# bistromath/gr-ais

Hardware: AMD Instinct MI355X
Metric: complex MS/s through corr_est->msk_timing chain; corr_est %HBM roofline (higher is better)
Workload: dtype f32

## Files before the change

__graft_entry__.py:

```python
import os
import subprocess
import sys

ROOT = os.path.dirname(os.path.abspath(__file__))
for _p in (ROOT, os.path.join(ROOT, "gr-ais_amd"), os.path.join(ROOT, "tests")):
    if _p not in sys.path:
        sys.path.insert(0, _p)


def build():
    env = dict(os.environ)
    subprocess.check_call(["make", "-C", os.path.join(ROOT, "gr-ais_amd")], env=env)
    subprocess.check_call(["make", "-C", os.path.join(ROOT, "oracle")], env=env)
    subprocess.check_call(["make", "-C", os.path.join(ROOT, "tests", "emul")], env=env)
    subprocess.check_call(["make", "-C", os.path.join(ROOT, "tests", "emul_hdlc")], env=env)
    subprocess.check_call(["make", "-C", os.path.join(ROOT, "tests", "emul_nmea")], env=env)
    subprocess.check_call(["make", "-C", os.path.join(ROOT, "tests", "emul_msg")], env=env)
    subprocess.check_call(["make", "-C", os.path.join(ROOT, "tests", "emul_xlate")], env=env)
    subprocess.check_call(["make", "-C", os.path.join(ROOT, "tests", "emul_xlate_fmt")], env=env)
    ub = os.path.join(ROOT, "tools", "ubench")
    src, exe = os.path.join(ub, "hbm_ceiling.hip"), os.path.join(ub, "hbm_ceiling")
    if not os.path.exists(exe) or os.path.getmtime(exe) < os.path.getmtime(src):
        subprocess.check_call([os.environ.get("HIPCC", "/opt/rocm/bin/hipcc"), "--offload-arch=gfx950", "-O3", "-o", exe, src], env=env)
    import ais_amd
    from ais_amd import _lib

    assert _lib.lib().aisx_version() >= 300


def smoke():
    import numpy as np
    import torch

    assert torch.cuda.is_available(), "smoke() needs cuda:0"
    import ais_amd
    import oracle_py as orc
    import synth
    from parity import assert_tags_match

    sps, nchan, T = 4, 8, 8192
    tmpl = ais_amd.modulate_vector_bc(ais_amd.gmsk_mod(sps, 0.4), [1, 1, 0, 0] * 7, [1])
    xs = np.stack([synth.make_channel(31 + c, T, "S", sps, amp=1.0, cfo_max=10.0)[0] for c in range(nchan)])
    opts = dict(samples_per_symbol=sps, bits_per_sec=9600.0, clockrec_gain=0.04, omega_relative_limit=0.01,
                fftlen=1024)
    dem = ais_amd.ais_demod(opts, nchan=nchan, max_items=T, stages="core", preamble_symbols=tmpl)
    r = dem.work(torch.as_tensor(xs).cuda())
    prod = r["produced"].cpu().numpy()
    bits = r["bits"].cpu().numpy()
    tags = dem.preamble_detect.tags()
    ndet = 0
    for c in range(nchan):
        ob, _, ot = orc.Demod(sps, tmpl, stages=0).step(xs[c])
        ndet += assert_tags_match(tags[tags["chan"] == c], ot)
        assert prod[c] == len(ob) and np.array_equal(bits[c, : prod[c]], ob)
    fs = ais_amd.square_and_fft_sync_cc(38400.0, 9600.0, 1024, nchan=nchan, max_items=T)
    agc = ais_amd.feedforward_agc_cc(512, 2.0, nchan=nchan, max_items=T + 1024)
    y = ais_amd.freq_sync_agc(fs, agc, torch.as_tensor(xs).cuda())[0].cpu().numpy()
    for c in range(nchan):
        yo, _ = orc.FreqSync(38400.0, 9600.0, 1024).process(xs[c])
        assert np.array_equal(y[c].view(np.uint32), orc.Agc(512, 2.0).work(yo).view(np.uint32))
    print("smoke ok: %d channels, %d detections, %d bits and %d front-end samples identical to the oracle"
          % (nchan, ndet, int(prod.sum()), y.size))


if __name__ == "__main__":
    build()
    if len(sys.argv) > 1 and sys.argv[1] == "smoke":
        smoke()
```

gr-ais_amd/csrc/k_msk.h:

```cpp
#pragma once
#include "aisx_common.h"

namespace aisx {

enum {
    MSK_ST_INTERP_RANGE = 1,
    MSK_ST_CARRY_OVERFLOW = 2,
    MSK_ST_TAGCARRY_OVERFLOW = 4,
    MSK_ST_OUT_FULL = 8,
    MSK_ST_TAGS_TRUNCATED = 16
};
constexpr int MSK_CTN_TRUNC = 0x40000000;
constexpr int MSK_CTN_WILD = 0x20000000;
constexpr int MSK_TAG_TRIPS = 6;

constexpr int MSK_T = 64;
constexpr int MSK_RING = 256;
constexpr int MSK_SLOTS = MSK_RING + 8;
constexpr int MSK_CHUNK = 64;
constexpr int MSK_OFF = 192;
constexpr int MSK_CARRY_MAX = 128;
constexpr int MSK_PAIRS_MAX = 16;
constexpr int MSK_TAPS_PITCH = 12;
constexpr int msk_lds_ring(int lpw) { return MSK_SLOTS * lpw * 8; }
constexpr int MSK_ZERO_ROW = 129;
constexpr int MSK_LDS_MMSE = ((130 * MSK_TAPS_PITCH * 4 + 511) / 512) * 512;
constexpr int MSK_TAGQ = 36;
#ifndef MSK_WAVES_LPW4
#define MSK_WAVES_LPW4 4
#endif
constexpr int msk_waves(int lpw) { return lpw >= 16 ? 64 / lpw : (lpw == 4 ? MSK_WAVES_LPW4 : 4); }
constexpr int msk_wg_channels(int lpw) { return msk_waves(lpw) * lpw; }
constexpr int MSK_STAGE = 32;
static_assert(MSK_STAGE >= 15 + MSK_PAIRS_MAX + 1, "a lock-step run and a general step between two flushes");
constexpr bool msk_staged(int lpw) { return lpw <= 8; }
constexpr int msk_lds_stage(int lpw) { return msk_staged(lpw) ? MSK_STAGE * lpw * 8 : 0; }
constexpr int msk_lds_ringoff(int lpw) { return msk_waves(lpw) * msk_lds_stage(lpw); }
constexpr int msk_lds_wave(int lpw) { return msk_lds_ring(lpw) + MSK_TAGQ * lpw * 8 + lpw * 8; }
constexpr int msk_lds_taboff(int lpw) { return msk_lds_ringoff(lpw) + msk_waves(lpw) * msk_lds_wave(lpw); }
constexpr int msk_lds_bytes(int lpw) { return msk_lds_taboff(lpw) + MSK_LDS_MMSE; }
static_assert(msk_lds_bytes(4) <= 160 * 1024 && msk_lds_bytes(8) <= 160 * 1024 && msk_lds_bytes(16) <= 160 * 1024 &&
              msk_lds_bytes(32) <= 160 * 1024 && msk_lds_bytes(64) <= 160 * 1024, "a workgroup's LDS");
static_assert(msk_lds_bytes(8) + 71680 <= 160 * 1024, "timing recovery + one correlator workgroup per CU");
constexpr int BT_T = 256;
constexpr int BT_SEG = BT_T * 8;

constexpr int MSKP_SMAX = 64;
enum { MSKP_KIND_NONE = 0, MSKP_KIND_NEXT = 1, MSKP_KIND_HANDOFF = 2 };
struct mskp_rst {
    int jA;
    int relA, relB;
    int q0, cap;
    int pad[3];
};
struct mskp_snap {
    int a;
    float mu, omega;
    int div;
    cf y;
    cf nl;
    int cur;
    int cnt;
};
struct mskp_res {
    mskp_snap end;
    cf ay, anl;
    int kind;
    int status;
};
struct mskp_piece {
    int out0, src0, cnt;
};
AISX_HD bool mskp_same_bits(cf a, cf b)
{
    unsigned ar, ai, br, bi;
    __builtin_memcpy(&ar, &a.re, 4);
    __builtin_memcpy(&ai, &a.im, 4);
    __builtin_memcpy(&br, &b.re, 4);
    __builtin_memcpy(&bi, &b.im, 4);
    return ar == br && ai == bi;
}

struct msk_ctag { int rel; float val; };

struct __attribute__((packed, aligned(8))) cf_pair { cf a, b; };

struct MskParams {
    int nchan;
    float d_sps, gain, gain_omega, limit;
    int osps;
    float* mu; float* omega; int* div;
    cf* dly1; cf* dly2; cf* diff1;
    unsigned long long* nread;
    const cf* in; long in_stride; int n;
    const cf* carry_in; cf* carry_out; const int* carry_len_in; int* carry_len_out; int carry_cap;
    int stream_mode; int gr_ninput; int gr_noutput;
    const msk_ctag* ct; const int* ct_n; int ct_cap;
    tag_rec* ctag_out; int* ctag_n_out; int ctag_cap;
    cf* syms; float* err; float* mu_out; long out_stride; int out_cap;
    int* produced; int* consumed; int* status;
    const float* mmse;
    int lds_tab_off;
    int lds_wave_stride, tq_stride, tq_private;
    int lds_ring_off;
    int sym_al16;
    int lpw;
    int inline_tags;
    int max_noutput;
    int ff;
    const int* nrst; const mskp_rst* rst; const mskp_res* res;
    mskp_piece* pieces; int* npieces;
    const int* ct_nc;
};

struct BitTailParams {
    int nchan;
    const cf* syms; long sym_stride;
    const int* produced;
    unsigned char* bits; long bit_stride;
    const cf* prev_sym_in; const unsigned char* prev_bit_in;
    cf* prev_sym_out; unsigned char* prev_bit_out;
    const float* atan_tab;
};

AISX_HD int msk_forecast(float d_sps, int noutput_items)
{
    return (int)ceil((noutput_items * d_sps * 2) + 3.0 * d_sps + 8u);
}

#ifdef MSK_EMU_STATS
extern long msk_stats[8];
#endif
template <class Ctx, bool AUX, bool OSPS2, int LPW, bool FFT = false>
AISX_DI void msk_body(Ctx& cx, const MskParams& p)
{
    static_assert(!FFT || (!AUX && !OSPS2), "the join build has no err / mu ports and osps == 1");
    constexpr int SLOT_B = LPW * 8;
    constexpr int SLOT_SH = LPW == 64 ? 9 : (LPW == 32 ? 8 : (LPW == 16 ? 7 : (LPW == 8 ? 6 : 5)));
    static_assert(LPW == 4 || LPW == 8 || LPW == 16 || LPW == 32 || LPW == 64, "channels per wave");
    typedef unsigned long long u64;
    static_assert(64 % LPW == 0, "whole waves");
    constexpr int NQ = 64 / LPW;
    constexpr int QS = MSK_CHUNK / NQ;
    const int wv = cx.tid() >> 6;
    const int l = cx.tid() & (LPW - 1);
    const int q = (cx.tid() & 63) / LPW;
    const bool owner = q == 0;
    const int cbase = cx.bx() * msk_wg_channels(LPW) + wv * LPW;
    const int c = cbase + l;
    const bool live = c < p.nchan;
    const int cc = live ? c : (p.nchan - 1);

    char* const lds0 = cx.lds();
    char* const lds = lds0 + p.lds_ring_off + wv * p.lds_wave_stride;
    cf* ring = (cf*)lds;
    float* mm = (float*)(lds0 + p.lds_tab_off);
    cf* myring = ring + l;

    for (int i = cx.tid(); i < 129 * 8; i += cx.nthreads())
        mm[(i >> 3) * MSK_TAPS_PITCH + (i & 7)] = p.mmse[i];
    if (cx.tid() < MSK_TAPS_PITCH)
        mm[MSK_ZERO_ROW * MSK_TAPS_PITCH + cx.tid()] = 0.f;
    if (cbase >= p.nchan) {
        cx.sync();
        return;
    }

    const float d_sps = p.d_sps;
    float d_mu = p.mu[cc], d_omega = p.omega[cc];
    int d_div = p.div[cc];
    cf last_interp = p.dly1[cc];
    cf d_dly_diff_1 = p.diff1[cc];
    cf prev_sq = cmul_exact(p.dly2[cc], p.dly2[cc]);
    const unsigned long long R = p.nread[cc];
    int status = 0;
    const int n = p.n;

    const cf* cin = p.carry_in + (long)cc * p.carry_cap;
    int pending = p.carry_len_in[cc];
    if (pending > MSK_CARRY_MAX)
        pending = MSK_CARRY_MAX;
    const int navail = pending + n;
    for (int q = -1; q < pending; q++) {
        const int slot = (q - pending + MSK_OFF) & (MSK_RING - 1);
        myring[slot * LPW] = cin[q + 1];
        if (slot < 8)
            myring[(MSK_RING + slot) * LPW] = cin[q + 1];
    }

    const msk_ctag* ctl = p.ct + (long)cc * p.ct_cap;
    int ntot = p.ct_n[cc];
    if (ntot & MSK_CTN_TRUNC)
        status |= MSK_ST_TAGS_TRUNCATED;
    const bool tame_tags = p.inline_tags && cx.ballot((ntot & MSK_CTN_WILD) != 0) == 0ull;
    ntot &= MSK_CTN_WILD - 1;
    if (ntot > p.ct_cap)
        ntot = p.ct_cap;
    typedef msk_ctag tq_ent;
    tq_ent* const tq = (tq_ent*)(lds + msk_lds_ring(LPW)) + (p.tq_private ? (cx.tid() & 63) : l);
    const int TQS = p.tq_stride;
    const int TQ_NONE = 0x7fffffff;
    int gq = 0;
    int qhead = 0, qn = 0;
    auto tq_fill = [&]() {
        if (qn > 0) {
            tq[0] = tq[(qn - 1) * TQS];
            qn = 1;
        }
        qhead = qn;
        while (qn < MSK_TAGQ && gq < ntot) {
            tq_ent t[4];
#pragma unroll
            for (int j = 0; j < 4; j++)
                t[j] = ctl[gq + j < ntot ? gq + j : ntot - 1];
#pragma unroll
            for (int j = 0; j < 4; j++) {
                if (qn < MSK_TAGQ && gq < ntot) {
                    gq++;
                    tq[qn * TQS] = t[j];
                    qn++;
                }
            }
        }
    };
    int fr_rel = TQ_NONE;
    float nt_val = 0.f;
    int nt_rel = 0x7fffffff;
    auto tq_front = [&]() {
        if (qhead >= qn && gq < ntot)
            tq_fill();
        if (qhead < qn) {
            const tq_ent e = tq[qhead * TQS];
            fr_rel = e.rel;
            nt_val = e.val;
        } else {
            fr_rel = TQ_NONE;
        }
    };
    auto tq_pop = [&]() {
        qhead++;
        tq_front();
    };
    tq_fill();

    constexpr bool FF = FFT;
    bool fin_saved = false;
    float fin_mu = 0.f, fin_omega = 0.f;
    int fin_div = 0, fin_status = 0;
    cf fin_interp = mk(0.f, 0.f), fin_diff = mk(0.f, 0.f);
    unsigned fin_worst = 0;
    int ffK = 0, ffnck = 0, cand = 0, candj = 0x7fffffff, ffnp = 0;
    int voff = 0;
    const mskp_rst* const ffrs = FF ? p.rst + (long)cc * MSKP_SMAX : nullptr;
    const mskp_res* const ffrr = FF ? p.res + (long)cc * MSKP_SMAX : nullptr;
    if (FF) {
        ffnck = p.ct_nc[cc];
        ffK = ffnck >= 0 ? p.nrst[cc] : 0;
        candj = ffK > 0 ? ffrs[0].jA + 1 + ffnck : 0x7fffffff;
    }

    char* const osym0 = (char*)(p.syms + (long)cbase * p.out_stride);
    char* const oerr0 = AUX && p.err ? (char*)(p.err + (long)cbase * p.out_stride) : nullptr;
    char* const omu0 = AUX && p.mu_out ? (char*)(p.mu_out + (long)cbase * p.out_stride) : nullptr;
    unsigned ob = (unsigned)((long)(cc - cbase) * p.out_stride) * 8u;
    constexpr bool STG = !AUX && !OSPS2 && msk_staged(LPW);
    constexpr unsigned FLQ = NQ < 8 ? NQ : 8;
    constexpr unsigned FL = 2 * FLQ;
    constexpr unsigned STG_MASK = (unsigned)((MSK_STAGE - 1) * SLOT_B);
    const unsigned obrow = ob;
    const unsigned stg_real = (unsigned)(wv * msk_lds_stage(LPW) + l * 8);
    const unsigned stg_spare = (unsigned)(p.lds_ring_off + wv * p.lds_wave_stride + p.lds_wave_stride - SLOT_B + l * 8);
    unsigned so = 0;
    unsigned nf = 0;
    struct alignas(8) cf8s { float re, im; };
    auto stage_put = [&](unsigned mask, unsigned base, cf v) {
        cf8s t;
        t.re = v.re;
        t.im = v.im;
        *(cf8s*)(lds0 + ((so & mask) | base)) = t;
        so += (unsigned)SLOT_B;
    };
    auto stage_get = [&](unsigned k) -> cf {
        const cf8s t = *(const cf8s*)(lds0 + ((((k & (unsigned)(MSK_STAGE - 1)) << SLOT_SH)) | stg_real));
        return mk(t.re, t.im);
    };
    auto flush_syms = [&]() {
        if constexpr (STG) {
            if (cx.ballot((so >> SLOT_SH) - nf >= FL) == 0ull)
                return;
            cx.wave_sync();
            while (cx.ballot((so >> SLOT_SH) - nf >= FL) != 0ull) {
                if ((so >> SLOT_SH) - nf >= FL) {
                    const unsigned k0 = nf + 2u * (unsigned)q;
                    if ((NQ <= 8 || (unsigned)q < FLQ) && !fin_saved) {
                        const cf a = stage_get(k0), b = stage_get(k0 + 1u);
                        cf* dst = (cf*)(osym0 + obrow) + k0;
                        if (p.sym_al16) {
                            st16(dst, a, b);
                        } else {
                            st8(dst, a);
                            st8(dst + 1, b);
                        }
                    }
                    nf += FL;
                }
            }
            cx.wave_sync();
        }
    };

    int base = 0, ototal = 0;
    int iidx = 0, oidx = 0;
    int ninp = 0, noutput = 0;
    bool done = false;
    auto setup_round = [&]() {
        int ninput;
        if (p.stream_mode) {
            ninput = (navail - base) - 1;
            noutput = 0;
            if (ninput > 0) {
                noutput = (int)((ninput - 3.0 * d_sps - 8) / (2.0 * d_sps)) + 2;
                while (noutput > 0 && msk_forecast(d_sps, noutput) > ninput)
                    noutput--;
            }
            if (p.max_noutput > 0 && noutput > p.max_noutput)
                noutput = p.max_noutput;
            if (noutput > p.out_cap - ototal) {
                noutput = p.out_cap - ototal;
                status |= MSK_ST_OUT_FULL;
            }
        } else {
            ninput = p.gr_ninput;
            noutput = p.gr_noutput;
        }
        ninp = (int)(ninput - 3.0 * d_sps);
        iidx = 0;
        oidx = 0;
        if (ninp <= 0 || noutput <= 0) {
            done = true;
            return;
        }
        qhead = 0;
        tq_front();
        while (fr_rel < base)
            tq_pop();
        nt_rel = (fr_rel != TQ_NONE && fr_rel - base < ninp) ? fr_rel - base : 0x7fffffff;
    };
    if (!done)
        setup_round();
    const int jump_margin = (int)ceilf(d_sps) + 1;

    const int nchunks = (n + 8 + MSK_CHUNK - 1) / MSK_CHUNK;
    cf r[QS];
    const cf* myin = p.in + (long)cc * p.in_stride;
    auto issue_chunk = [&](int t) {
        const int s0 = t * MSK_CHUNK + q * QS + voff;
        const bool inside = FF ? cx.ballot(!(s0 >= 0 && t * MSK_CHUNK + MSK_CHUNK + voff <= n)) == 0ull : (t * MSK_CHUNK + MSK_CHUNK <= n);
        if (inside) {
            const cf_pair* src = (const cf_pair*)(myin + s0);
#pragma unroll
            for (int k = 0; k < QS / 2; k++) {
                const cf_pair v = src[k];
                r[2 * k] = v.a;
                r[2 * k + 1] = v.b;
            }
        } else {
#pragma unroll
            for (int k = 0; k < QS; k++) {
                r[k] = mk(0.f, 0.f);
                if (s0 + k < n && s0 + k >= 0)
                    r[k] = myin[s0 + k];
            }
        }
    };
    auto land_chunk = [&](int t) {
        const int slot0 = (t * MSK_CHUNK + MSK_OFF) & (MSK_RING - 1);
#pragma unroll
        for (int k = 0; k < QS; k++)
            myring[(slot0 + q * QS + k) * LPW] = r[k];
        if (slot0 == 0 && q * QS < 8) {
#pragma unroll
            for (int k = 0; k < (QS < 8 ? QS : 8); k++)
                myring[(MSK_RING + q * QS + k) * LPW] = r[k];
        }
    };
    issue_chunk(0);
    land_chunk(0);
    int landed = 1;
    cx.sync();

    int sb = (base + iidx - pending + MSK_OFF) * SLOT_B;
    int fast_lim = (int)0x80000000;
    int tag_trig = (int)0x80000000;
    unsigned worst_imu = 0;
    bool more = false;
    int loaded_s = 0;
    enum { EV_PARK = 0, EV_GO = 1, EV_OTHER_PARITY = 2 };
    const int TRIG_FORCED = (int)0x80000001;

    auto bounds = [&](int spos) {
        tag_trig = 0x7fffffff;
        if (nt_rel != 0x7fffffff && iidx <= nt_rel) {
            int i = nt_rel - jump_margin - 1;
            while (!((float)nt_rel < ((float)i + d_sps)))
                i++;
            tag_trig = i;
        }
        const int chunk_lim = more ? (loaded_s - 8 - jump_margin + MSK_OFF - (spos - iidx) + 1) : 0x7fffffff;
        fast_lim = ninp < tag_trig ? ninp : tag_trig;
        fast_lim = fast_lim < chunk_lim ? fast_lim : chunk_lim;
    };
    auto ff_walk = [&]() -> bool {
        bool moved = false;
        int dcnt = 0, a_new = 0, cur_new = 0;
        int oidx_w = oidx, nout_w = noutput, otot_w = ototal;
        bool crossed = false;
        cf yv = last_interp, nlv = d_dly_diff_1;
        float mu_new = 0.f, om_new = 0.f;
        int div_new = 0;
        const int cd = jump_margin - 1;
        for (;;) {
            const mskp_res r = ffrr[cand];
            const bool same = r.kind != MSKP_KIND_NONE && mskp_same_bits(r.ay, yv) && mskp_same_bits(r.anl, nlv);
            bool clean = same && (r.end.a + 1 + cd <= base + ninp - pending) && ffnp < MSKP_SMAX;
            if (p.max_noutput > 0 && r.kind == MSKP_KIND_NEXT)
                clean = clean && msk_forecast(d_sps, p.max_noutput) <= (n - r.end.a) - 1 &&
                        (ototal + oidx + dcnt + r.end.cnt + p.max_noutput <= p.out_cap);
            else
                clean = clean && (oidx_w + r.end.cnt < nout_w);
            if (!clean) {
                cand++;
                candj = cand < ffK ? ffrs[cand].jA + 1 + ffnck : 0x7fffffff;
                break;
            }
            if (owner && live) {
                mskp_piece pc;
                pc.out0 = ototal + oidx + dcnt;
                pc.src0 = ffrs[cand].q0;
                pc.cnt = r.end.cnt;
                p.pieces[(long)cc * MSKP_SMAX + ffnp] = pc;
            }
            ffnp++;
            moved = true;
            dcnt += r.end.cnt;
            oidx_w += r.end.cnt;
            while (p.max_noutput > 0 && oidx_w >= nout_w) {
                oidx_w -= nout_w;
                otot_w += nout_w;
                nout_w = p.max_noutput;
                crossed = true;
            }
            a_new = r.end.a;
            mu_new = r.end.mu;
            om_new = r.end.omega;
            div_new = r.end.div;
            yv = r.end.y;
            nlv = r.end.nl;
            cur_new = r.end.cur;
            status |= r.status;
            cand++;
            candj = cand < ffK ? ffrs[cand].jA + 1 + ffnck : 0x7fffffff;
            if (r.kind == MSKP_KIND_NEXT && cand < ffK)
                continue;
            break;
        }
        if (!moved)
            return false;
        if constexpr (STG) {
            if (owner) {
                for (unsigned kk = nf; kk < (so >> SLOT_SH); kk++)
                    st8((cf*)(osym0 + obrow) + kk, stage_get(kk));
            }
            nf = (so >> SLOT_SH) + (unsigned)dcnt;
            so += (unsigned)dcnt << SLOT_SH;
        }
        ob += (unsigned)dcnt * 8u;
        d_mu = mu_new;
        d_omega = om_new;
        d_div = div_new;
        last_interp = yv;
        prev_sq = cmul_exact(yv, yv);
        d_dly_diff_1 = nlv;
        gq = cur_new + ffnck;
        if (gq > ntot)
            gq = ntot;
        qn = 0;
        qhead = 0;
        tq_fill();
        const int q_new = a_new + pending;
        tq_front();
        if (crossed) {
            ototal = otot_w;
            base = (fr_rel != TQ_NONE && fr_rel < q_new) ? fr_rel : q_new;
            setup_round();
        } else {
            nt_rel = (fr_rel != TQ_NONE && fr_rel - base < ninp) ? fr_rel - base : 0x7fffffff;
        }
        iidx = q_new - base;
        oidx = oidx_w;
        const int v_new = loaded_s - MSK_CHUNK + 1;
        voff = a_new - v_new;
        sb = (v_new + MSK_OFF) * SLOT_B;
        {
            const int slot0 = (loaded_s - MSK_CHUNK + MSK_OFF) & (MSK_RING - 1);
            constexpr int SH = Ctx::wave_lds_coherent ? 1 : NQ;
            for (int sh = 0; sh < SH; sh++) {
                const int k0 = ((Ctx::wave_lds_coherent ? q : sh) * QS);
                cf t[QS];
#pragma unroll
                for (int k = 0; k < QS; k++) {
                    const int sr = loaded_s - MSK_CHUNK + k0 + k + voff;
                    t[k] = mk(0.f, 0.f);
                    if (sr >= 0 && sr < n)
                        t[k] = myin[sr];
                }
#pragma unroll
                for (int k = 0; k < QS; k++) {
                    myring[(slot0 + k0 + k) * LPW] = t[k];
                    if (slot0 == 0 && k0 + k < 8)
                        myring[(MSK_RING + k0 + k) * LPW] = t[k];
                }
            }
            if (more) {
                const int s0 = landed * MSK_CHUNK + q * QS + voff;
#pragma unroll
                for (int k = 0; k < QS; k++) {
                    r[k] = mk(0.f, 0.f);
                    if (s0 + k < n && s0 + k >= 0)
                        r[k] = myin[s0 + k];
                }
            }
        }
        tag_trig = (int)0x80000000;
        fast_lim = (int)0x80000000;
        return true;
    };
    auto events = [&](const int PAR) -> int {
        if (!(oidx < noutput && iidx < ninp)) {
            base += iidx;
            ototal += oidx;
            const bool progress = iidx > 0;
            if (!p.stream_mode || !progress)
                done = true;
            else
                setup_round();
        }
        if (done)
            return EV_PARK;
        const int spos = sb >> SLOT_SH;
        const bool waiting = more && !(spos - MSK_OFF + 8 + jump_margin <= loaded_s);
        if (!waiting && (nt_rel >= iidx) && ((float)nt_rel < ((float)iidx + d_sps))) {
            if (FF) {
                const int fi = gq - (qn - qhead);
                while (cand < ffK && candj < fi) {
                    cand++;
                    candj = cand < ffK ? ffrs[cand].jA + 1 + ffnck : 0x7fffffff;
                }
                if (cand < ffK && fi == candj && ff_walk()) {
                    bounds(sb >> SLOT_SH);
                    return EV_OTHER_PARITY;
                }
            }
            const float center = nt_val;
            if (center == center) {
                const int old = iidx;
                d_mu = center;
                iidx = nt_rel;
                if (d_mu < 0) {
                    d_mu++;
                    iidx--;
                }
                sb += (iidx - old) * SLOT_B;
                d_div = 0;
                d_omega = d_sps;
            }
            tq_pop();
            nt_rel = (fr_rel != TQ_NONE && fr_rel - base < ninp) ? fr_rel - base : 0x7fffffff;
            bounds(sb >> SLOT_SH);
            if (fast_lim <= iidx) {
                tag_trig = TRIG_FORCED;
                fast_lim = iidx + 1;
            }
            return ((d_div & 1) == PAR) ? EV_GO : EV_OTHER_PARITY;
        }
        bounds(spos);
        if (waiting)
            return EV_PARK;
        return EV_GO;
    };

    auto tap_row = [&](float mu) -> unsigned {
        const unsigned imu = (unsigned)(int)rintf(mu * 128.0f);
        return imu < (unsigned)MSK_ZERO_ROW ? imu : (unsigned)MSK_ZERO_ROW;
    };
    auto fir_load = [&](unsigned row, int sbpos, cf* sv, float* tv) {
        typedef float tap4 __attribute__((vector_size(16)));
        const tap4* tp4 = (const tap4*)((const char*)mm + row * (unsigned)(MSK_TAPS_PITCH * 4));
        const tap4 tlo = tp4[0], thi = tp4[1];
        const float tp[8] = { tlo[0], tlo[1], tlo[2], tlo[3], thi[0], thi[1], thi[2], thi[3] };
        struct alignas(8) cf8 { float re, im; };
        const cf8* sp = (const cf8*)(lds + (((unsigned)sbpos & (unsigned)((MSK_RING - 1) * SLOT_B)) | (unsigned)(l * 8)));
#pragma unroll
        for (int k = 0; k < 8; k++) {
            const cf8 t = sp[k * LPW];
            sv[k] = mk(t.re, t.im);
            tv[k] = tp[7 - k];
        }
    };
    const unsigned mm_rbase = mmse_row_base((unsigned)p.lds_tab_off, (unsigned)(MSK_TAPS_PITCH * 4));
    const char* const lds_l = lds + l * 8;
    constexpr unsigned RING_M = (unsigned)((MSK_RING - 1) * SLOT_B);
    auto fir_load_pair = [&](float mu, unsigned soff, cf* sv, float* tv) {
        typedef float tap4 __attribute__((vector_size(16)));
        const tap4* tp4 = (const tap4*)(lds0 + mmse_row_off(mu, (unsigned)(MSK_TAPS_PITCH * 4), mm_rbase));
        const tap4 tlo = tp4[0], thi = tp4[1];
        const float tp[8] = { tlo[0], tlo[1], tlo[2], tlo[3], thi[0], thi[1], thi[2], thi[3] };
        struct alignas(8) cf8 { float re, im; };
        const cf8* sp = (const cf8*)(lds_l + soff);
#pragma unroll
        for (int k = 0; k < 8; k++) {
            const cf8 t = sp[k * LPW];
            sv[k] = mk(t.re, t.im);
            tv[k] = tp[7 - k];
        }
    };
    auto fir_sum = [&](const cf* sv, const float* tv) -> cf {
        cf acc = mk(0.f, 0.f);
#pragma unroll
        for (int k = 0; k < 8; k++) {
            acc.re += sv[k].re * tv[k];
            acc.im += sv[k].im * tv[k];
        }
        return acc;
    };

    auto fir = [&](unsigned row, int sbpos) -> cf {
        cf sv[8];
        float tv[8];
        fir_load(row, sbpos, sv, tv);
        return fir_sum(sv, tv);
    };

    auto body = [&](const int PAR) {
        const unsigned row = tap_row(d_mu);
        worst_imu = worst_imu > row ? worst_imu : row;
        const cf in_interp = fir(row, sb);
        const cf sq = cmul_exact(in_interp, in_interp);
        const cf dly_conj = cconj(prev_sq);
        const cf nlin_out = cmul_exact(sq, dly_conj);
        float err_out = (nlin_out - d_dly_diff_1).re;
        if (PAR) {
            err_out = branchless_clip(err_out, 3.0f);
            d_omega += p.gain_omega * err_out;
            d_omega = d_sps + branchless_clip(d_omega - d_sps, p.limit);
            d_mu += p.gain * err_out;
        }
        if (!PAR || OSPS2) {
            if constexpr (STG)
                stage_put(STG_MASK, stg_real, in_interp);
            else
                *(cf*)(osym0 + ob) = in_interp;
            if (AUX) {
                if (oerr0)
                    *(float*)(oerr0 + (ob >> 1)) = err_out;
                if (omu0)
                    *(float*)(omu0 + (ob >> 1)) = d_mu;
            }
            ob += 8u;
            oidx++;
        }
        d_div++;
        last_interp = in_interp;
        prev_sq = sq;
        d_dly_diff_1 = nlin_out;
        d_mu += d_omega;
        const float fl = floorf(d_mu);
        const int adv = (int)fl;
        iidx += adv;
        sb += adv * SLOT_B;
        d_mu = d_mu - fl;
    };

#ifdef MSK_PROF
    long long pf_t0 = __builtin_readcyclecounter(), pf_lock = 0, pf_land = 0, pf_gen = 0, pf_n[4] = {0, 0, 0, 0}, pf_fail = 0, pf_nfail = 0;
#define PF_BEGIN long long pf_a = __builtin_readcyclecounter();
#define PF_END(acc) acc += __builtin_readcyclecounter() - pf_a;
#else
#define PF_BEGIN
#define PF_END(acc)
#endif
    u64 P = 0;
    u64 E = 0;
    auto ok_for = [&](const int PAR) -> bool {
        return (PAR || OSPS2) ? ((iidx < fast_lim) && (oidx < noutput)) : (iidx < fast_lim);
    };

    auto step = [&](const int PAR) {
        const u64 mine = ~P & (PAR ? ~E : E);
        const u64 okM = cx.ballot(ok_for(PAR));
        u64 goM = mine & okM;
        const u64 evM = mine & ~okM;
        if (evM != 0ull) {
#ifdef MSK_PROF
            pf_n[3]++;
#endif
            int code = -1;
            if (cx.inv_ballot(evM))
                code = events(PAR);
            goM |= cx.ballot(code == EV_GO);
            P |= cx.ballot(code == EV_PARK);
            E = cx.ballot((d_div & 1) == 0);
        }
        if (goM != 0ull) {
            if (cx.inv_ballot(goM))
                body(PAR);
            E ^= goM;
        }
    };

    const u64 ALL = cx.ballot(true);

    const float wmax = d_sps + fabsf(p.limit);
    const float pair_adv = 2.0f * wmax + 3.0f * fabsf(p.gain);
    const float pair_adv_inv = 0.9999f / pair_adv;
    const bool lock_ok = 3.0f * fabsf(p.gain) + fabsf(p.limit) + 0.01f < d_sps;
    auto rearm = [&]() {
        const int chunk_lim = more ? (loaded_s - 8 - jump_margin + MSK_OFF - ((sb >> SLOT_SH) - iidx) + 1) : 0x7fffffff;
        int f = ninp < tag_trig ? ninp : tag_trig;
        f = f < chunk_lim ? f : chunk_lim;
        fast_lim = (tag_trig == TRIG_FORCED) ? fast_lim : f;
    };
    auto need_more = [&]() -> bool {
        return FF ? cx.ballot(!done && landed * MSK_CHUNK < n + 8 - voff) != 0ull : landed < nchunks;
    };
    more = need_more();
    if (more)
        issue_chunk(landed);
    loaded_s = landed * MSK_CHUNK;
    P = cx.ballot(done);
    E = cx.ballot((d_div & 1) == 0);
    rearm();
    for (;;) {
        flush_syms();
        const u64 DN = FF ? cx.ballot(done) : 0ull;
        if (FF && done && !fin_saved) {
            fin_saved = true;
            fin_mu = d_mu;
            fin_omega = d_omega;
            fin_div = d_div;
            fin_interp = last_interp;
            fin_diff = d_dly_diff_1;
            fin_status = status;
            fin_worst = worst_imu;
            if constexpr (STG) {
                if (owner) {
                    for (unsigned kk = nf; kk < (so >> SLOT_SH); kk++)
                        st8((cf*)(osym0 + obrow) + kk, stage_get(kk));
                }
                nf = so >> SLOT_SH;
            }
        }
        { PF_BEGIN
        if ((P & ~DN) == 0ull && (E | DN) == ALL && DN != ALL) {
            const float room = fast_lim > iidx ? (float)(fast_lim - iidx) - (1.001f + wmax) : -1.f;
            int can = room >= 0.f ? (int)(room * pair_adv_inv) + 1 : 0;
            can = can < MSK_PAIRS_MAX ? can : MSK_PAIRS_MAX;
            const int ocan = OSPS2 ? (noutput - oidx) / 2 : (noutput - oidx) - 1;
            can = can < ocan ? can : ocan;
            if (!lock_ok || !(d_mu >= 0.f && d_mu <= 1.f))
                can = 0;
            int npairs = 0;
            if ((cx.ballot(can >= 1) | DN) == ALL) {
                npairs = MSK_PAIRS_MAX;
                if ((cx.ballot(can >= MSK_PAIRS_MAX) | DN) != ALL) {
                    npairs = 1;
                    for (int bit = MSK_PAIRS_MAX / 2; bit; bit >>= 1)
                        if (npairs + bit < MSK_PAIRS_MAX && (cx.ballot(can >= npairs + bit) | DN) == ALL)
                            npairs += bit;
                }
            }
            if constexpr (NQ >= 2 && !AUX && !OSPS2) {
              if (npairs == 0 && tame_tags) {
                constexpr int ROW = LPW <= 16 ? 16 : 32;
                const int chunk_lim2 = more ? (loaded_s - 8 - jump_margin + MSK_OFF - ((sb >> SLOT_SH) - iidx) + 1) : 0x7fffffff;
                const int lim2 = ninp < chunk_lim2 ? ninp : chunk_lim2;
                const float room2 = lim2 > iidx ? (float)(lim2 - iidx) - (1.001f + wmax + d_sps) : -1.f;
                int can2 = room2 >= 0.f ? (int)(room2 * (0.9999f / (pair_adv + d_sps))) + 1 : 0;
                can2 = can2 < MSK_TAG_TRIPS ? can2 : MSK_TAG_TRIPS;
                can2 = can2 < ocan ? can2 : ocan;
                if (!lock_ok || !(d_mu >= 0.f && d_mu <= 1.f) || tag_trig == TRIG_FORCED)
                    can2 = 0;
                int ntrips = 0;
                if ((cx.ballot(can2 >= 1) | DN) == ALL) {
                    ntrips = 1;
                    while (ntrips < MSK_TAG_TRIPS && (cx.ballot(can2 >= ntrips + 1) | DN) == ALL)
                        ntrips++;
                }
                if (ntrips > 0) {
                    const bool roleO = (cx.tid() & ROW) != 0;
                    const unsigned rstep = (unsigned)(cx.tid() & ROW) * (unsigned)(SLOT_B / ROW);
                    const unsigned pmask = roleO ? 0u : STG_MASK, pbase = roleO ? stg_spare : stg_real;
                    cf sqO = prev_sq, sqE = mk(0.f, 0.f), acc = last_interp;
                    float nl_prev = d_dly_diff_1.re;
                    bool last_skip = false;
                    for (int k = 0; k < ntrips; k++) {
#ifdef MSK_EMU_STATS
                        if (l == 0 && q == 0) msk_stats[5]++;
#endif
                        const bool fireE = (nt_rel >= iidx) && ((float)nt_rel < ((float)iidx + d_sps));
                        if (cx.ballot(fireE) != 0ull) {
                            if (fireE) {
                                const float center = nt_val;
                                if (center == center) {
                                    int at = nt_rel;
                                    float m = center;
                                    if (m < 0) {
                                        m++;
                                        at--;
                                    }
                                    sb += (at - iidx) * SLOT_B;
                                    iidx = at;
                                    d_mu = m;
                                    d_div = 0;
                                    d_omega = d_sps;
                                }
                                tq_pop();
                                nt_rel = (fr_rel != TQ_NONE && fr_rel - base < ninp) ? fr_rel - base : 0x7fffffff;
                            }
                        }
                        const float m1 = d_mu + d_omega;
                        const float muO = cx.fract(m1);
                        const int adv1 = (int)m1;
                        const int sb1 = sb + adv1 * SLOT_B;
                        const int iidxO = iidx + adv1;
                        const bool winO = (nt_rel >= iidxO) && ((float)nt_rel < ((float)iidxO + d_sps));
                        const bool nanO = winO && (nt_val != nt_val);
                        if (cx.ballot(nanO) != 0ull) {
                            if (nanO) {
                                tq_pop();
                                nt_rel = (fr_rel != TQ_NONE && fr_rel - base < ninp) ? fr_rel - base : 0x7fffffff;
                            }
                        }
                        const bool skipO = winO && !nanO;
                        cf sv[8];
                        float tv[8];
                        fir_load_pair(roleO ? muO : d_mu, ring_read_off(sb, adv1, rstep, RING_M), sv, tv);
                        acc = fir_sum(sv, tv);
                        const cf sq = cmul_exact(acc, acc);
                        cf sE, s1;
                        cx.template pair_rows<ROW>(sq, sE, s1);
                        const float nlE = sE.re * sqO.re + sE.im * sqO.im;
                        const float nlO = s1.re * sE.re + s1.im * sE.im;
                        const float err = branchless_clip(nlO - nlE, 3.0f);
                        float om2 = d_omega + p.gain_omega * err;
                        om2 = d_sps + branchless_clip(om2 - d_sps, p.limit);
                        const float mu2 = muO + p.gain * err;
                        if constexpr (STG) {
                            stage_put(pmask, pbase, acc);
                        } else {
                            if (!roleO)
                                *(cf*)(osym0 + ob) = acc;
                            ob += 8u;
                        }
                        const float m2 = mu2 + om2;
                        const int adv2 = (int)m2;
                        d_mu = skipO ? muO : cx.fract(m2);
                        sb = skipO ? sb1 : sb1 + adv2 * SLOT_B;
                        iidx = skipO ? iidxO : iidxO + adv2;
                        d_omega = skipO ? d_omega : om2;
                        d_div += skipO ? 1 : 2;
                        const cf nE = skipO ? sqO : sE, nO = skipO ? sE : s1;
                        sqE = nE;
                        sqO = nO;
                        nl_prev = skipO ? nlE : nlO;
                        last_skip = skipO;
                    }
                    cf accE, accO;
                    cx.template pair_rows<ROW>(acc, accE, accO);
                    oidx += ntrips;
                    prev_sq = sqO;
                    last_interp = last_skip ? accE : accO;
                    d_dly_diff_1 = mk(nl_prev, sqO.im * sqE.re - sqO.re * sqE.im);
                    if (!(d_mu >= 0.f && d_mu <= 1.f))
                        status |= MSK_ST_INTERP_RANGE;
                    E = cx.ballot((d_div & 1) == 0);
                    bounds(sb >> SLOT_SH);
#ifdef MSK_PROF
                    pf_n[0] += ntrips; pf_n[1]++;
#endif
                }
              }
            }
#ifdef MSK_PROF
            if (npairs == 0) { pf_fail += __builtin_readcyclecounter() - pf_a; pf_nfail++; }
#endif
            if (npairs > 0) {
              if constexpr (NQ >= 2) {
                constexpr int ROW = LPW <= 16 ? 16 : 32;
                const bool roleO = (cx.tid() & ROW) != 0;
                const unsigned rstep = (unsigned)(cx.tid() & ROW) * (unsigned)(SLOT_B / ROW);
                const unsigned pmask = roleO ? 0u : STG_MASK, pbase = roleO ? stg_spare : stg_real;
                cf sqO = prev_sq, sqE = mk(0.f, 0.f), acc = last_interp;
                float nl_prev = d_dly_diff_1.re;
                const int sb_entry = sb;
                for (int k = 0; k < npairs; k++) {
#ifdef MSK_EMU_STATS
                    if (l == 0 && q == 0) msk_stats[0]++;
#endif
                    const float m1 = d_mu + d_omega;
                    const float muO = cx.fract(m1);
                    const int adv1 = (int)m1;
                    const int sb1 = sb + adv1 * SLOT_B;
                    cf sv[8];
                    float tv[8];
                    fir_load_pair(roleO ? muO : d_mu, ring_read_off(sb, adv1, rstep, RING_M), sv, tv);
                    acc = fir_sum(sv, tv);
                    const cf sq = cmul_exact(acc, acc);
                    cf sE, s1;
                    cx.template pair_rows<ROW>(sq, sE, s1);
                    const float nlE = sE.re * sqO.re + sE.im * sqO.im;
                    const float nlO = s1.re * sE.re + s1.im * sE.im;
                    const float err = branchless_clip(nlO - nlE, 3.0f);
                    d_omega += p.gain_omega * err;
                    d_omega = d_sps + branchless_clip(d_omega - d_sps, p.limit);
                    const float mu2 = muO + p.gain * err;
                    if (OSPS2) {
                        const unsigned o = ob + (roleO ? 8u : 0u);
                        *(cf*)(osym0 + o) = acc;
                        if (AUX) {
                            if (oerr0)
                                *(float*)(oerr0 + (o >> 1)) = roleO ? err : nlE - nl_prev;
                            if (omu0)
                                *(float*)(omu0 + (o >> 1)) = roleO ? mu2 : d_mu;
                        }
                        ob += 16u;
                    } else if constexpr (STG) {
                        stage_put(pmask, pbase, acc);
                    } else {
                        if (!roleO) {
                            *(cf*)(osym0 + ob) = acc;
                            if (AUX) {
                                if (oerr0)
                                    *(float*)(oerr0 + (ob >> 1)) = nlE - nl_prev;
                                if (omu0)
                                    *(float*)(omu0 + (ob >> 1)) = d_mu;
                            }
                        }
                        ob += 8u;
                    }
                    const float m2 = mu2 + d_omega;
                    d_mu = cx.fract(m2);
                    sb = sb1 + (int)m2 * SLOT_B;
                    sqE = sE;
                    sqO = s1;
                    nl_prev = nlO;
                }
                cf accE, accO;
                cx.template pair_rows<ROW>(acc, accE, accO);
                d_div += 2 * npairs;
                oidx += OSPS2 ? 2 * npairs : npairs;
                iidx += (sb - sb_entry) >> SLOT_SH;
                prev_sq = sqO;
                last_interp = accO;
                d_dly_diff_1 = mk(nl_prev, sqO.im * sqE.re - sqO.re * sqE.im);
                if (!(d_mu >= 0.f && d_mu <= 1.f))
                    status |= MSK_ST_INTERP_RANGE;
              } else {
                const int sb_entry = sb;
                cf sqO = prev_sq, sqE = mk(0.f, 0.f), accO = last_interp;
                float nl_prev = d_dly_diff_1.re;
                for (int k = 0; k < npairs; k++) {
#ifdef MSK_EMU_STATS
                    if (l == 0) msk_stats[0]++;
#endif
                    cf svE[8], svO[8];
                    float tvE[8], tvO[8];
                    fir_load_pair(d_mu, (unsigned)sb & RING_M, svE, tvE);
                    const float m1 = d_mu + d_omega;
                    const float muO = cx.fract(m1);
                    const int sb1 = sb + (int)m1 * SLOT_B;
                    fir_load_pair(muO, (unsigned)sb1 & RING_M, svO, tvO);
                    const cf accE = fir_sum(svE, tvE);
                    const cf sE = cmul_exact(accE, accE);
                    const float nlE = sE.re * sqO.re + sE.im * sqO.im;
                    if constexpr (STG)
                        stage_put(STG_MASK, stg_real, accE);
                    else
                        *(cf*)(osym0 + ob) = accE;
                    if (AUX) {
                        if (oerr0)
                            *(float*)(oerr0 + (ob >> 1)) = nlE - nl_prev;
                        if (omu0)
                            *(float*)(omu0 + (ob >> 1)) = d_mu;
                    }
                    ob += 8u;
                    const cf acc1 = fir_sum(svO, tvO);
                    const cf s1 = cmul_exact(acc1, acc1);
                    const float nlO = s1.re * sE.re + s1.im * sE.im;
                    const float err = branchless_clip(nlO - nlE, 3.0f);
                    d_omega += p.gain_omega * err;
                    d_omega = d_sps + branchless_clip(d_omega - d_sps, p.limit);
                    const float mu2 = muO + p.gain * err;
                    if (OSPS2) {
                        *(cf*)(osym0 + ob) = acc1;
                        if (AUX) {
                            if (oerr0)
                                *(float*)(oerr0 + (ob >> 1)) = err;
                            if (omu0)
                                *(float*)(omu0 + (ob >> 1)) = mu2;
                        }
                        ob += 8u;
                    }
                    const float m2 = mu2 + d_omega;
                    d_mu = cx.fract(m2);
                    sb = sb1 + (int)m2 * SLOT_B;
                    sqE = sE;
                    sqO = s1;
                    accO = acc1;
                    nl_prev = nlO;
                }
                d_div += 2 * npairs;
                oidx += OSPS2 ? 2 * npairs : npairs;
                iidx += (sb - sb_entry) >> SLOT_SH;
                prev_sq = sqO;
                last_interp = accO;
                d_dly_diff_1 = mk(nl_prev, sqO.im * sqE.re - sqO.re * sqE.im);
                if (!(d_mu >= 0.f && d_mu <= 1.f))
                    status |= MSK_ST_INTERP_RANGE;
              }
#ifdef MSK_PROF
                pf_n[0] += npairs; pf_n[1]++;
#endif
            }
        }
        PF_END(pf_lock) }
        { PF_BEGIN
        if (FF && !more) {
            more = need_more();
            if (more)
                issue_chunk(landed);
        }
        if (more) {
            const bool clear = done || ((sb >> SLOT_SH) - MSK_OFF >= landed * MSK_CHUNK - (MSK_RING - MSK_CHUNK) + 2);
            if (cx.ballot(clear) == ALL) {
#ifdef MSK_EMU_STATS
                if (l == 0) msk_stats[4]++;
#endif
                cx.wave_sync();
                land_chunk(landed);
                cx.wave_sync();
                landed++;
                more = need_more();
                if (more)
                    issue_chunk(landed);
                loaded_s = landed * MSK_CHUNK;
                P = cx.ballot(done);
                rearm();
                if (P == 0ull && E == ALL) {
                    PF_END(pf_land)
                    continue;
                }
            }
        }
        PF_END(pf_land) }
#ifdef MSK_EMU_STATS
        if (l == 0) { msk_stats[1]++; if (P != 0ull) msk_stats[2]++; if (E != ALL && E != 0ull) msk_stats[3]++; }
#endif
        { PF_BEGIN
        step(0);
        step(1);
#ifdef MSK_PROF
        pf_n[2]++;
#endif
        PF_END(pf_gen) }
        if (P == ALL && (!more || cx.ballot(done) == ALL))
            break;
    }

#ifdef MSK_PROF
    if (c == 0 && owner) {
        long long pf_t1 = __builtin_readcyclecounter();
        printf("msk prof: total %lld lock %lld (failed entries %lld: %lld) land %lld gen %lld | pairs %lld runs %lld genpasses %lld events %lld\n", pf_t1 - pf_t0, pf_lock, pf_nfail, pf_fail, pf_land, pf_gen, pf_n[0], pf_n[1], pf_n[2], pf_n[3]);
    }
#endif
    if constexpr (STG) {
        flush_syms();
        const unsigned left = fin_saved ? 0u : (so >> SLOT_SH) - nf;
#pragma unroll
        for (unsigned j = 0; j < 2; j++) {
            const unsigned k = (unsigned)q + j * FLQ;
            if ((unsigned)q < FLQ && k < left)
                st8((cf*)(osym0 + obrow) + nf + k, stage_get(nf + k));
        }
    }
    if (!live || !owner)
        return;
    if (fin_saved) {
        d_mu = fin_mu;
        d_omega = fin_omega;
        d_div = fin_div;
        last_interp = fin_interp;
        d_dly_diff_1 = fin_diff;
        status = fin_status;
        worst_imu = fin_worst;
    }
    if (worst_imu >= (unsigned)MSK_ZERO_ROW)
        status |= MSK_ST_INTERP_RANGE;
    p.mu[c] = d_mu;
    p.omega[c] = d_omega;
    p.div[c] = d_div;
    p.dly1[c] = last_interp;
    p.dly2[c] = last_interp;
    p.diff1[c] = d_dly_diff_1;
    const unsigned long long Rn = R + (unsigned long long)base;
    p.nread[c] = Rn;
    p.produced[c] = ototal;
    p.consumed[c] = base;

    cf* cout = p.carry_out + (long)c * p.carry_cap;
    if (p.stream_mode) {
        int left = navail - base;
        int cap = p.carry_cap < MSK_CARRY_MAX ? p.carry_cap : MSK_CARRY_MAX;
        if (left + 1 > cap) {
            status |= MSK_ST_CARRY_OVERFLOW;
            left = cap - 1;
        }
        if (FF) {
            for (int k = 0; k <= left; k++) {
                const int qi = base - 1 + k;
                cout[k] = qi < pending ? cin[qi + 1] : myin[qi - pending];
            }
            p.npieces[c] = ffnp;
        } else {
            for (int k = 0; k <= left; k++)
                cout[k] = myring[((base - 1 + k - pending + MSK_OFF) & (MSK_RING - 1)) * LPW];
        }
        p.carry_len_out[c] = left;
        tag_rec* cto = p.ctag_out + (long)c * p.ctag_cap;
        int w = 0;
        for (int k = 0; k < qn; k++) {
            const tq_ent e = tq[k * TQS];
            if (e.rel < base)
                continue;
            if (w < p.ctag_cap) {
                tag_rec tg;
                tg.offset = R + (unsigned long long)e.rel;
                tg.value = (double)e.val;
                tg.key = KEY_TIME_EST;
                tg.chan = c;
                cto[w] = tg;
            } else {
                status |= MSK_ST_TAGCARRY_OVERFLOW;
            }
            w++;
        }
        for (int k = gq; k < ntot; k++) {
            const tq_ent e = ctl[k];
            if (e.rel < base)
                continue;
            if (w < p.ctag_cap) {
                tag_rec tg;
                tg.offset = R + (unsigned long long)e.rel;
                tg.value = (double)e.val;
                tg.key = KEY_TIME_EST;
                tg.chan = c;
                cto[w] = tg;
            } else {
                status |= MSK_ST_TAGCARRY_OVERFLOW;
            }
            w++;
        }
        p.ctag_n_out[c] = w < p.ctag_cap ? w : p.ctag_cap;
    } else {
        cout[0] = myring[((base - 1 - pending + MSK_OFF) & (MSK_RING - 1)) * LPW];
        p.carry_len_out[c] = 0;
        p.ctag_n_out[c] = 0;
    }
    p.status[c] = status;
}

struct TagPrepParams {
    int nchan;
    const tag_rec* ctag_in; const int* ctag_n_in; int ctag_cap;
    const tag_rec* tags; const int* tag_count; int tag_cap;
    const unsigned long long* nread;
    msk_ctag* ct; int* ct_n; int ct_cap;
    int* ct_nc;
    const msk_ctag* ctl_new; const int* ctl_new_n; int ctl_new_cap; int ctl_new_pre; unsigned long long W;
};

template <class Ctx>
AISX_DI void tagprep_body(Ctx& cx, const TagPrepParams& p)
{
    const int l = cx.tid() & 63;
    const int c = cx.bx() * (cx.nthreads() >> 6) + (cx.tid() >> 6);
    if (c >= p.nchan)
        return;
    const unsigned long long R = p.nread[c];
    msk_ctag* out = p.ct + (long)c * p.ct_cap;
    int w = 0;
    bool wild = false;
    auto scan = [&](const tag_rec* list, int n) {
        for (int k0 = 0; k0 < n; k0 += 64) {
            const int k = k0 + l;
            tag_rec t;
            t.offset = 0;
            t.value = 0;
            t.key = -1;
            if (k < n)
                t = list[k];
            const bool keep = (k < n) && t.key == KEY_TIME_EST && t.offset >= R;
            const float tv = (float)t.value;
            if (cx.ballot(keep && !(tv != tv) && !(tv >= -1.0f && tv <= 1.0f)) != 0ull)
                wild = true;
            const unsigned long long m = cx.ballot(keep);
            const int pos = w + aisx_popc64(m & ((1ull << l) - 1ull));
            if (keep && pos < p.ct_cap) {
                const unsigned long long d = t.offset - R;
                msk_ctag e;
                e.rel = d > 0x7ffffff0ull ? 0x7ffffff0 : (int)d;
                e.val = (float)t.value;
                out[pos] = e;
            }
            w += aisx_popc64(m);
        }
    };
    bool trunc = false;
    int nc = p.ctag_n_in[c];
    if (nc > p.ctag_cap)
        nc = p.ctag_cap;
    scan(p.ctag_in + (long)c * p.ctag_cap, nc);
    const int kept_carried = w;
    bool newdrop = false;
    if (p.ctl_new) {
        int nn = p.ctl_new_n[c];
        if (nn & MSK_CTN_TRUNC)
            trunc = true;
        if (nn & MSK_CTN_WILD)
            wild = true;
        nn &= MSK_CTN_WILD - 1;
        const msk_ctag* list = p.ctl_new + (long)c * p.ctl_new_cap + p.ctl_new_pre;
        const long long shift = (long long)(p.W - R);
        for (int k0 = 0; k0 < nn; k0 += 64) {
            const int k = k0 + l;
            msk_ctag e;
            e.rel = 0;
            e.val = 0.f;
            if (k < nn)
                e = list[k];
            const long long d = shift + (long long)e.rel;
            const bool keep = (k < nn) && d >= 0;
            if (cx.ballot((k < nn) && !keep) != 0ull)
                newdrop = true;
            const unsigned long long m = cx.ballot(keep);
            const int pos = w + aisx_popc64(m & ((1ull << l) - 1ull));
            if (keep && pos < p.ct_cap) {
                msk_ctag o;
                o.rel = d > 0x7ffffff0ll ? 0x7ffffff0 : (int)d;
                o.val = e.val;
                out[pos] = o;
            }
            w += aisx_popc64(m);
        }
    } else if (p.tags) {
        int nn = p.tag_count[c];
        if (nn > p.tag_cap) {
            nn = p.tag_cap;
            trunc = true;
        }
        const int w0 = w;
        scan(p.tags + (long)c * p.tag_cap, nn);
        if (p.ct_nc) {
            int nkey = 0;
            const tag_rec* list = p.tags + (long)c * p.tag_cap;
            for (int k0 = 0; k0 < nn; k0 += 64) {
                const int k = k0 + l;
                nkey += aisx_popc64(cx.ballot(k < nn && list[k].key == KEY_TIME_EST));
            }
            newdrop = (w - w0) != nkey;
        }
    }
    if (w > p.ct_cap)
        trunc = true;
    if (l == 0) {
        p.ct_n[c] = (w < p.ct_cap ? w : p.ct_cap) | (trunc ? MSK_CTN_TRUNC : 0) | (wild ? MSK_CTN_WILD : 0);
        if (p.ct_nc)
            p.ct_nc[c] = (newdrop || trunc) ? -1 : kept_carried;
    }
}

template <class Ctx>
AISX_DI void bittail_body(Ctx& cx, const BitTailParams& p)
{
    const int ch = cx.by();
    const int t = cx.tid();
    float* at = (float*)cx.lds();
    for (int i = t; i < 257; i += BT_T)
        at[i] = p.atan_tab[i];
    cx.sync();
    const int P = p.produced[ch];
    const cf* sy = p.syms + (long)ch * p.sym_stride;
    unsigned char* ob = p.bits + (long)ch * p.bit_stride;
    const cf sym_m1 = p.prev_sym_in[ch];
    const unsigned char bit_m1 = p.prev_bit_in[ch];
    auto slice = [&](const cf& cur, const cf& prev) -> unsigned char {
        const cf prod = cmul_exact(cur, cconj(prev));
        const float y = prod.im, x = prod.re;
        const float ya = fabsf(y), xa = fabsf(x);
        const bool plain = (ya < 1.0e30f) && (xa < 1.0e18f) && (y >= 0.0f || ya > 1.0e-18f);
        if (plain)
            return y >= 0.0f ? 1 : 0;
        const float fm = 1.57079632679489661923f * fast_atan2f_tab(y, x, at);
        return fm >= 0 ? 1 : 0;
    };
    if (cx.bx() == 0 && t == 0 && P == 0) {
        p.prev_sym_out[ch] = sym_m1;
        p.prev_bit_out[ch] = bit_m1;
    }
    const int o0 = cx.bx() * BT_SEG;
    for (int k = 0; k < BT_SEG / BT_T; k++) {
        const int o = o0 + k * BT_T + t;
        if (o >= P)
            break;
        const cf s0 = sy[o];
        const cf s1 = o >= 1 ? sy[o - 1] : sym_m1;
        const unsigned char b = slice(s0, s1);
        unsigned char bp = bit_m1;
        if (o >= 1)
            bp = slice(s1, o >= 2 ? sy[o - 2] : sym_m1);
        const unsigned char d = (unsigned char)(((unsigned)(b - bp)) % 2u);
        ob[o] = (unsigned char)((d ^ 0x01) & 0x01);
        if (o == P - 1) {
            p.prev_sym_out[ch] = s0;
            p.prev_bit_out[ch] = b;
        }
    }
}

}
```

Before: 47290.

## Skip idle MSK steps, gate flushes, and add fast path for tag-free trips

The MSK timing-recovery loop now calls the symbol flush only when a flag says new symbols were staged. `step` returns early when no lanes in the wave are eligible. The tagged lock-step entry is gated by a wave ballot on whether a tag triggered the limit. Inside tagged runs, trips where no lane is near a tag take a plain pair-update path that skips the per-trip tag checks. The goal is to cut wave-wide ballots, syncs and branchy tag handling in the hot loop, at the cost of more flag bookkeeping that could delay a flush if it is missed.

```diff
diff --git a/__graft_entry__.py b/__graft_entry__.py
--- a/__graft_entry__.py
+++ b/__graft_entry__.py
@@ -13,6 +13,7 @@
     subprocess.check_call(["make", "-C", os.path.join(ROOT, "gr-ais_amd")], env=env)
     subprocess.check_call(["make", "-C", os.path.join(ROOT, "oracle")], env=env)
     subprocess.check_call(["make", "-C", os.path.join(ROOT, "tests", "emul")], env=env)
+    subprocess.check_call(["make", "-C", os.path.join(ROOT, "tests", "emul_msk_state")], env=env)
     subprocess.check_call(["make", "-C", os.path.join(ROOT, "tests", "emul_hdlc")], env=env)
     subprocess.check_call(["make", "-C", os.path.join(ROOT, "tests", "emul_nmea")], env=env)
     subprocess.check_call(["make", "-C", os.path.join(ROOT, "tests", "emul_msg")], env=env)
diff --git a/gr-ais_amd/csrc/k_msk.h b/gr-ais_amd/csrc/k_msk.h
--- a/gr-ais_amd/csrc/k_msk.h
+++ b/gr-ais_amd/csrc/k_msk.h
@@ -284,11 +284,23 @@
         const cf8s t = *(const cf8s*)(lds0 + ((((k & (unsigned)(MSK_STAGE - 1)) << SLOT_SH)) | stg_real));
         return mk(t.re, t.im);
     };
+#ifdef MSK_PROF
+    long long pf_t0 = __builtin_readcyclecounter(), pf_lock = 0, pf_land = 0, pf_gen = 0, pf_n[9] = {0, 0, 0, 0, 0, 0, 0, 0, 0}, pf_fail = 0, pf_nfail = 0;
+    long long pf_tag = 0, pf_flush = 0;
+#define PF_BEGIN long long pf_a = __builtin_readcyclecounter();
+#define PF_END(acc) acc += __builtin_readcyclecounter() - pf_a;
+#else
+#define PF_BEGIN
+#define PF_END(acc)
+#endif
     auto flush_syms = [&]() {
         if constexpr (STG) {
             if (cx.ballot((so >> SLOT_SH) - nf >= FL) == 0ull)
                 return;
             cx.wave_sync();
+#ifdef MSK_PROF
+            pf_n[7]++;
+#endif
             while (cx.ballot((so >> SLOT_SH) - nf >= FL) != 0ull) {
                 if ((so >> SLOT_SH) - nf >= FL) {
                     const unsigned k0 = nf + 2u * (unsigned)q;
@@ -681,14 +693,7 @@
         d_mu = d_mu - fl;
     };
 
-#ifdef MSK_PROF
-    long long pf_t0 = __builtin_readcyclecounter(), pf_lock = 0, pf_land = 0, pf_gen = 0, pf_n[4] = {0, 0, 0, 0}, pf_fail = 0, pf_nfail = 0;
-#define PF_BEGIN long long pf_a = __builtin_readcyclecounter();
-#define PF_END(acc) acc += __builtin_readcyclecounter() - pf_a;
-#else
-#define PF_BEGIN
-#define PF_END(acc)
-#endif
+    bool fl_due = true;
     u64 P = 0;
     u64 E = 0;
     auto ok_for = [&](const int PAR) -> bool {
@@ -697,6 +702,8 @@
 
     auto step = [&](const int PAR) {
         const u64 mine = ~P & (PAR ? ~E : E);
+        if (mine == 0ull)
+            return;
         const u64 okM = cx.ballot(ok_for(PAR));
         u64 goM = mine & okM;
         const u64 evM = mine & ~okM;
@@ -715,6 +722,8 @@
             if (cx.inv_ballot(goM))
                 body(PAR);
             E ^= goM;
+            if (!PAR || OSPS2)
+                fl_due = true;
         }
     };
 
@@ -741,7 +750,10 @@
     E = cx.ballot((d_div & 1) == 0);
     rearm();
     for (;;) {
-        flush_syms();
+        if (fl_due) { PF_BEGIN
+            flush_syms();
+            fl_due = false;
+        PF_END(pf_flush) }
         const u64 DN = FF ? cx.ballot(done) : 0ull;
         if (FF && done && !fin_saved) {
             fin_saved = true;
@@ -761,6 +773,9 @@
             }
         }
         { PF_BEGIN
+#ifdef MSK_PROF
+        bool pf_tagged = false;
+#endif
         if ((P & ~DN) == 0ull && (E | DN) == ALL && DN != ALL) {
             const float room = fast_lim > iidx ? (float)(fast_lim - iidx) - (1.001f + wmax) : -1.f;
             int can = room >= 0.f ? (int)(room * pair_adv_inv) + 1 : 0;
@@ -780,7 +795,7 @@
                 }
             }
             if constexpr (NQ >= 2 && !AUX && !OSPS2) {
-              if (npairs == 0 && tame_tags) {
+              if (npairs == 0 && tame_tags && cx.ballot(can == 0 && fast_lim == tag_trig) != 0ull) {
                 constexpr int ROW = LPW <= 16 ? 16 : 32;
                 const int chunk_lim2 = more ? (loaded_s - 8 - jump_margin + MSK_OFF - ((sb >> SLOT_SH) - iidx) + 1) : 0x7fffffff;
                 const int lim2 = ninp < chunk_lim2 ? ninp : chunk_lim2;
@@ -803,10 +818,54 @@
                     cf sqO = prev_sq, sqE = mk(0.f, 0.f), acc = last_interp;
                     float nl_prev = d_dly_diff_1.re;
                     bool last_skip = false;
+                    const unsigned nearw = (unsigned)((int)ceilf(wmax + d_sps) + 2);
                     for (int k = 0; k < ntrips; k++) {
 #ifdef MSK_EMU_STATS
                         if (l == 0 && q == 0) msk_stats[5]++;
 #endif
+                        if (cx.ballot((unsigned)nt_rel - (unsigned)iidx < nearw) == 0ull) {
+#ifdef MSK_EMU_STATS
+                            if (l == 0 && q == 0) msk_stats[6]++;
+#endif
+#ifdef MSK_PROF
+                            pf_n[8]++;
+#endif
+                            const float m1 = d_mu + d_omega;
+                            const float muO = cx.fract(m1);
+                            const int adv1 = (int)m1;
+                            const int sb1 = sb + adv1 * SLOT_B;
+                            cf sv[8];
+                            float tv[8];
+                            fir_load_pair(roleO ? muO : d_mu, ring_read_off(sb, adv1, rstep, RING_M), sv, tv);
+                            acc = fir_sum(sv, tv);
+                            const cf sq = cmul_exact(acc, acc);
+                            cf sE, s1;
+                            cx.template pair_rows<ROW>(sq, sE, s1);
+                            const float nlE = sE.re * sqO.re + sE.im * sqO.im;
+                            const float nlO = s1.re * sE.re + s1.im * sE.im;
+                            const float err = branchless_clip(nlO - nlE, 3.0f);
+                            d_omega += p.gain_omega * err;
+                            d_omega = d_sps + branchless_clip(d_omega - d_sps, p.limit);
+                            const float mu2 = muO + p.gain * err;
+                            if constexpr (STG) {
+                                stage_put(pmask, pbase, acc);
+                            } else {
+                                if (!roleO)
+                                    *(cf*)(osym0 + ob) = acc;
+                                ob += 8u;
+                            }
+                            const float m2 = mu2 + d_omega;
+                            const int adv2 = (int)m2;
+                            d_mu = cx.fract(m2);
+                            sb = sb1 + adv2 * SLOT_B;
+                            iidx += adv1 + adv2;
+                            d_div += 2;
+                            sqE = sE;
+                            sqO = s1;
+                            nl_prev = nlO;
+                            last_skip = false;
+                            continue;
+                        }
                         const bool fireE = (nt_rel >= iidx) && ((float)nt_rel < ((float)iidx + d_sps));
                         if (cx.ballot(fireE) != 0ull) {
                             if (fireE) {
@@ -884,17 +943,19 @@
                     if (!(d_mu >= 0.f && d_mu <= 1.f))
                         status |= MSK_ST_INTERP_RANGE;
                     E = cx.ballot((d_div & 1) == 0);
+                    fl_due = true;
                     bounds(sb >> SLOT_SH);
 #ifdef MSK_PROF
-                    pf_n[0] += ntrips; pf_n[1]++;
+                    pf_n[4] += ntrips; pf_n[5]++; pf_tag += __builtin_readcyclecounter() - pf_a; pf_tagged = true;
 #endif
                 }
               }
             }
 #ifdef MSK_PROF
-            if (npairs == 0) { pf_fail += __builtin_readcyclecounter() - pf_a; pf_nfail++; }
+            if (npairs == 0 && !pf_tagged) { pf_fail += __builtin_readcyclecounter() - pf_a; pf_nfail++; }
 #endif
             if (npairs > 0) {
+              fl_due = true;
               if constexpr (NQ >= 2) {
                 constexpr int ROW = LPW <= 16 ? 16 : 32;
                 const bool roleO = (cx.tid() & ROW) != 0;
@@ -1050,6 +1111,9 @@
                 land_chunk(landed);
                 cx.wave_sync();
                 landed++;
+#ifdef MSK_PROF
+                pf_n[6]++;
+#endif
                 more = need_more();
                 if (more)
                     issue_chunk(landed);
@@ -1080,7 +1144,8 @@
 #ifdef MSK_PROF
     if (c == 0 && owner) {
         long long pf_t1 = __builtin_readcyclecounter();
-        printf("msk prof: total %lld lock %lld (failed entries %lld: %lld) land %lld gen %lld | pairs %lld runs %lld genpasses %lld events %lld\n", pf_t1 - pf_t0, pf_lock, pf_nfail, pf_fail, pf_land, pf_gen, pf_n[0], pf_n[1], pf_n[2], pf_n[3]);
+        printf("msk prof: total %lld lock %lld tagged %lld (failed entries %lld: %lld) land %lld gen %lld flush %lld | pairs %lld runs %lld trips %lld (plain %lld) tagruns %lld landings %lld genpasses %lld events %lld flushes %lld\n",
+               pf_t1 - pf_t0, pf_lock, pf_tag, pf_nfail, pf_fail, pf_land, pf_gen, pf_flush, pf_n[0], pf_n[1], pf_n[4], pf_n[8], pf_n[5], pf_n[6], pf_n[2], pf_n[3], pf_n[7]);
     }
 #endif
     if constexpr (STG) {
```

After: 47610, median of 6. No clear change (+0.7%).
